# carpedkm/disentangled-subject-to-vid

Measured on AMD Instinct MI355X. Metric: denoise steps/sec (CogVideoX-5B, 49f 720x480; one step = CFG-pair transformer forward + CFG + scheduler step), higher is better.
Workload: dtype bf16

## Files before the change

disentangled-subject-to-vid_amd/csrc/api.hip:

```cpp
#define S2V_HOST
#include "common.h"
#include "kernels.h"
#include "../../include/s2v_hip.h"

#include <algorithm>
#include <cstdio>
#include <cstring>
#include <string>
#include <unordered_map>
#include <vector>

thread_local std::string g_s2v_err;
int s2v_fail(const char* file, int line, const char* msg, int code) {
    char buf[512];
    snprintf(buf, sizeof(buf), "%s:%d: %s", file, line, msg);
    g_s2v_err = buf;
    return code;
}

static inline int64_t rup(int64_t x, int64_t m) { return (x + m - 1) / m * m; }

struct Slot {
    char* dst = nullptr;
    int64_t rows = 0, cols = 0, ld = 0;
// ... 558 lines not shown
                for (int64_t j = 0; j < n; ++j, ++i) { omap[i] = (int)((so + j * Dp) / 16); omap[Mg + i] = (int)((so + n * Dp) / 4 + j * (Dp / 128)); }
            c->xcnt[1][0][g] = o_bytes(n); c->xcnt[1][1][g] = so; so += c->xcnt[1][0][g];
            c->xcnt[1][2][g] = o_bytes(c->M); c->xcnt[1][3][g] = g * o_bytes(c->M);
            c->xcnt[2][0][g] = (int64_t)B * c->Vmax * Cout4 * E; c->xcnt[2][1][g] = 0;
            c->xcnt[2][2][g] = c->xcnt[2][0][g]; c->xcnt[2][3][g] = g * c->xcnt[2][0][g];
        }
        if (omx) S2V_CHECK_HIP(hipMemcpy(c->omap, omap.data(), omap.size() * 4, hipMemcpyHostToDevice));
    }
    return 0;
}

extern "C" int s2v_fp8_qk_active(s2v_ctx* c, int32_t* active) {
    S2V_REQUIRE(c && active, "s2v_fp8_qk_active: null argument");
    *active = c->fp8_qk ? 1 : 0;
    return 0;
}

extern "C" int s2v_set_rope(s2v_ctx* c, const float* cos_dev, const float* sin_dev, s2v_stream stream) {
    S2V_REQUIRE(c && c->ws, "s2v_set_rope: call s2v_set_geometry first");
    auto drop_graph = [&]() { if (c->gexec) { hipGraphExecDestroy(c->gexec); c->gexec = nullptr; } };
    if (!cos_dev || !sin_dev) {
        if (c->have_rope) drop_graph();
        c->have_rope = false;
        return 0;
    }
    const bool had_rope = c->have_rope, was_paired = c->rope_paired;
    const size_t bytes = (size_t)(c->R + c->V) * 64 * 4;
    if (c->shard) {
        const size_t row = 64 * 4, rb = (size_t)c->R * row, vb = (size_t)c->V * row;
        const size_t ro = (size_t)c->r0 * row, vo = ((size_t)c->gR + c->v0) * row;
        S2V_CHECK_HIP(hipMemcpyAsync(c->rope_cos, (const char*)cos_dev + ro, rb, hipMemcpyDeviceToDevice, (hipStream_t)stream));
        S2V_CHECK_HIP(hipMemcpyAsync(c->rope_sin, (const char*)sin_dev + ro, rb, hipMemcpyDeviceToDevice, (hipStream_t)stream));
        S2V_CHECK_HIP(hipMemcpyAsync((char*)c->rope_cos + rb, (const char*)cos_dev + vo, vb, hipMemcpyDeviceToDevice, (hipStream_t)stream));
        S2V_CHECK_HIP(hipMemcpyAsync((char*)c->rope_sin + rb, (const char*)sin_dev + vo, vb, hipMemcpyDeviceToDevice, (hipStream_t)stream));
    } else {
        S2V_CHECK_HIP(hipMemcpyAsync(c->rope_cos, cos_dev, bytes, hipMemcpyDeviceToDevice, (hipStream_t)stream));
        S2V_CHECK_HIP(hipMemcpyAsync(c->rope_sin, sin_dev, bytes, hipMemcpyDeviceToDevice, (hipStream_t)stream));
    }
    c->have_rope = true;
    const size_t n = (size_t)(c->R + c->V) * 64;
    std::vector<float> hc(n), hs(n), pk(n);
    S2V_CHECK_HIP(hipStreamSynchronize((hipStream_t)stream));
    S2V_CHECK_HIP(hipMemcpy(hc.data(), c->rope_cos, bytes, hipMemcpyDeviceToHost));
    S2V_CHECK_HIP(hipMemcpy(hs.data(), c->rope_sin, bytes, hipMemcpyDeviceToHost));
    bool paired = true;
    for (size_t i = 0; i < n && paired; i += 2) paired = hc[i] == hc[i + 1] && hs[i] == hs[i + 1];
    c->rope_paired = paired;
    if (!had_rope || was_paired != paired) drop_graph();
    if (paired) {
        for (size_t p = 0; p < n / 64; ++p)
            for (int k = 0; k < 32; ++k) {
                pk[p * 64 + k] = hc[p * 64 + 2 * k];
                pk[p * 64 + 32 + k] = hs[p * 64 + 2 * k];
            }
        S2V_CHECK_HIP(hipMemcpy(c->rope_pk, pk.data(), bytes, hipMemcpyHostToDevice));
    }
    return 0;
}

extern "C" int s2v_set_pos_embed(s2v_ctx* c, const void* table_dev, s2v_stream stream) {
    S2V_REQUIRE(c && c->ws, "s2v_set_pos_embed: call s2v_set_geometry first");
    if (!table_dev) { c->have_pos = false; return 0; }
    S2V_CHECK_HIP(hipMemcpyAsync(c->pos_tab, (const char*)table_dev + (size_t)c->v0 * c->D * c->esz, (size_t)c->V * c->D * c->esz,
                                 hipMemcpyDeviceToDevice, (hipStream_t)stream));
    c->have_pos = true;
    return 0;
}

static int linear(s2v_ctx* c, const GemmArgs& g0, int epi, hipStream_t st) {
    GemmArgs g = g0;
    g.clk = c->clk_cur;
    g.a_rows_padded = (int)(rup(g.M, 256));
    g.w_rows_padded = (int)(rup(g.N, 256));
    if ((c->mfma || c->h16) && g.K % 64 == 0 && g.lda % 8 == 0 && g.ldw % 8 == 0) {
        g.f16 = c->h16 ? 1 : 0;
        const GemmPlan p = gemm_plan(g, epi, c->num_cus, c->sk_tiles);
        g.tile = p.tile;
        if (p.splitk > 1) { g.splitk = p.splitk; g.sk_ws = c->sk_ws; g.sk_cnt = c->sk_cnt; }
        if (p.tail != GEMM_NONE) {
            GemmArgs gm = g, gt = g;
            gt.clk = nullptr;
            gm.M = p.m_main;
            gt.m_begin = p.m_main;
            S2V_CHECK_HIP(hipEventRecord(c->ev_fork, st));
            S2V_CHECK_HIP(hipStreamWaitEvent(c->side, c->ev_fork, 0));
            S2V_TRY(launch_gemm_bf16(gt, epi, c->side));
            S2V_CHECK_HIP(hipEventRecord(c->ev_join, c->side));
            S2V_TRY(launch_gemm_bf16(gm, epi, st));
            S2V_CHECK_HIP(hipStreamWaitEvent(st, c->ev_join, 0));
            return 0;
        }
        return launch_gemm_bf16(g, epi, st);
    }
    g.valu_only = c->cfg.force_simple;
    return launch_gemm_simple(g, epi, c->dtype, st);
}

static int linear_fp8(s2v_ctx* c, const GemmArgs& g0, int epi, const char* wq, const float* wscale, hipStream_t st, bool prequant = false) {
    GemmArgs g = g0;
    g.clk = c->clk_cur;
    g.a_scale = nullptr;
    if (!g.mx_a_s) {
        if (!prequant) S2V_TRY(launch_quant_rows_fp8(g.A, g.lda, g.M, g.K, c->aq, c->aq_scale, st));
        g.A = c->aq; g.a_scale = c->aq_scale;
    }
    g.lda = g.K; g.W = wq; g.ldw = g.K; g.w_scale = wscale;
    g.a_rows_padded = (int)rup(g.M, 256);
    g.w_rows_padded = (int)rup(g.N, 256);
    return launch_gemm_fp8(g, epi, st);
}

extern "C" int s2v_set_conditioning(s2v_ctx* c, const void* text_dev, const void* ref_latent_dev, s2v_stream stream) {
    S2V_REQUIRE(c && c->ws && c->finalized, "s2v_set_conditioning: geometry and weights must be set first");
    S2V_REQUIRE(text_dev && ref_latent_dev, "s2v_set_conditioning: null input");
    hipStream_t st = (hipStream_t)stream;
    const int D = c->D;
    const int TX = c->cfg.text_embed_dim;
    if (c->T > 0) {
        if (c->shard) {
            for (int b = 0; b < c->B; ++b)
                S2V_TRY(launch_convert2d((const char*)text_dev + ((int64_t)b * c->gT + c->t0) * TX * c->esz, c->dtype, TX,
                                         c->Hb + (int64_t)b * c->T * TX * c->esz, c->dtype, TX, c->T, TX, st));
        } else {
            S2V_TRY(launch_convert2d(text_dev, c->dtype, TX, c->Hb, c->dtype, TX, (int64_t)c->B * c->T, TX, st));
        }
        GemmArgs g{};
        g.A = c->Hb; g.lda = TX; g.W = c->text_w; g.ldw = TX; g.bias = c->text_b;
        g.C = c->e0; g.ldc = D; g.M = c->B * c->T; g.N = D; g.K = TX;
        S2V_TRY(linear(c, g, EPI_BIAS, st));
    }
    const int K = c->cfg.in_channels * 4;
    S2V_TRY(launch_patchify(ref_latent_dev, 0, 1, 1, c->cfg.in_channels, c->H, c->W, c->patches, c->dtype, st));
    GemmArgs g{};
    g.A = c->patches + (int64_t)c->r0 * K * c->esz; g.lda = K; g.W = c->patch_w; g.ldw = K; g.bias = c->patch_b;
    g.C = c->e1; g.ldc = D; g.M = c->R; g.N = D; g.K = K;
    if (c->R > 0) S2V_TRY(linear(c, g, EPI_BIAS, st));
    c->have_cond = true;
    return 0;
}

#ifdef S2V_DIAG
static int g_fp8_mx = 1;
extern "C" __attribute__((visibility("default"))) int s2v_set_fp8_mx(int on) { g_fp8_mx = on; return 0; }
static int g_fused_q8 = 1;
extern "C" __attribute__((visibility("default"))) int s2v_set_fused_q8(int on) { g_fused_q8 = on; return 0; }
static int g_fused_qk = 1;
extern "C" __attribute__((visibility("default"))) int s2v_set_fused_qk(int on) { g_fused_qk = on; return 0; }
extern "C" __attribute__((visibility("default"))) int s2v_diag_qkv_qknorm(const void* A, const void* W, const void* bias, const void* nq_w, const void* nq_b,
                                                                           const void* nk_w, const void* nk_b, const float* cs, void* C, int32_t M, int32_t D,
                                                                           int32_t K, int32_t tok_per_batch, int32_t text_len, float eps, s2v_stream stream) {
    S2V_REQUIRE(A && W && bias && C && nq_w && nq_b && nk_w && nk_b, "s2v_diag_qkv_qknorm: null argument");
    GemmArgs g{};
    g.A = A; g.lda = K; g.W = W; g.ldw = K; g.bias = bias; g.C = C; g.ldc = 3 * D; g.M = M; g.N = 3 * D; g.K = K;
    g.a_rows_padded = (int)rup(M, 256); g.w_rows_padded = (int)rup(3 * D, 256);
    g.tok_per_batch = tok_per_batch; g.text_len = text_len;
    g.qk_w[0] = nq_w; g.qk_b[0] = nq_b; g.qk_w[1] = nk_w; g.qk_b[1] = nk_b; g.qk_cs = cs; g.qk_D = D; g.qk_eps = eps;
    return launch_gemm_bf16(g, EPI_BIAS_QKNORM, (hipStream_t)stream);
}
#endif
static bool attn_mx_out(const s2v_ctx* c) {
    bool mx = c->fp8 && c->mfma && c->D % 128 == 0;
#ifdef S2V_DIAG
    mx = mx && g_fp8_mx;
#endif
    return mx;
}
static int run_attention(s2v_ctx* c, int l, hipStream_t st, bool prequant = false) {
    const LayerW& w = c->layers[l];
    const int D = c->D;
    GemmArgs g{};
    g.A = c->Xn; g.lda = D; g.W = w.wqkv; g.ldw = D; g.bias = w.bqkv;
// ... 909 lines not shown
```

disentangled-subject-to-vid_amd/csrc/gemm.hip:

```cpp
#define S2V_HOST
#include "common.h"
#include "kernels.h"
#include <type_traits>
#include <algorithm>
#include <cstdlib>

#include "gemm_epi.h"
#include "epi_dispatch.h"

#define BM 128
#define BN 128
#define BK 64
#define TILE_BYTES (BM * BK * 2)

__device__ __forceinline__ int64_t a_row_base(const GemmArgs& a, int m) {
    if (!a.conv) return (int64_t)m * a.lda;
    m = min(m, a.M - 1);
    const int hw = a.oH * a.oW;
    const int f = m / hw, rem = m - f * hw;
    const int y = rem / a.oW, x = rem - y * a.oW;
    const int cs = a.cstride > 1 ? a.cstride : 1;
    return (((int64_t)f * a.Hp + y * cs) * a.Wp + x * cs) * a.cin;
}
__device__ __forceinline__ int64_t a_k_off(const GemmArgs& a, int k) {
// ... 49 lines not shown
template <int EPI, typename T16 = bf16_t>
__global__ __launch_bounds__(256, 2) void gemm_bf16_128(const GemmArgs a, int tiles_m, int tiles_n) {
    extern __shared__ __attribute__((aligned(16))) char smem[];
    const int tid = threadIdx.x, lane = tid & 63, wave = tid >> 6;
    const int wm = wave >> 1, wn = wave & 1;

    const int nwg = gridDim.x, bid = blockIdx.x;
    const int q = nwg >> 3, r = nwg & 7, xcd = bid & 7, idx = bid >> 3;
    const int wg = (xcd < r ? xcd * (q + 1) : r * (q + 1) + (xcd - r) * q) + idx;
    const int GM = 8;
    const int per_group = GM * tiles_n;
    const int group = wg / per_group;
    const int first_m = group * GM;
    const int gsz = min(tiles_m - first_m, GM);
    const int in_g = wg - group * per_group;
    const int tile_m = first_m + in_g % gsz;
    const int tile_n = in_g / gsz;
    const int m0 = a.m_begin + tile_m * BM, n0 = tile_n * BN;

    const bf16_t* A = (const bf16_t*)a.A;
    const bf16_t* W = (const bf16_t*)a.W;

    f32x16 acc[2][2];
#pragma unroll
    for (int i = 0; i < 2; ++i)
#pragma unroll
        for (int j = 0; j < 2; ++j)
#pragma unroll
            for (int e = 0; e < 16; ++e) acc[i][j][e] = 0.f;

    const int nt = a.K / BK;
    int64_t rb[4];
#pragma unroll
    for (int i = 0; i < 4; ++i) rb[i] = a_row_base(a, m0 + ((i * 256 + tid) >> 3));
    stage_tile_a(A, rb, a_k_off(a, 0), smem, tid);
    stage_tile(W, a.ldw, n0, 0, smem + TILE_BYTES, tid);
    __syncthreads();

    const int fr = lane & 31, hi = lane >> 5;
    for (int t = 0; t < nt; ++t) {
        const int cur = t & 1;
        if (t + 1 < nt) {
            stage_tile_a(A, rb, a_k_off(a, (t + 1) * BK), smem + (cur ^ 1) * 2 * TILE_BYTES, tid);
            stage_tile(W, a.ldw, n0, (t + 1) * BK, smem + (cur ^ 1) * 2 * TILE_BYTES + TILE_BYTES, tid);
        }
        const char* tA = smem + cur * 2 * TILE_BYTES;
        const char* tW = tA + TILE_BYTES;
#pragma unroll
        for (int kk = 0; kk < 4; ++kk) {
            bf16x8 wf[2], af[2];
#pragma unroll
            for (int i = 0; i < 2; ++i) wf[i] = lds_frag(tW, wn * 64 + i * 32 + fr, kk * 2 + hi);
#pragma unroll
            for (int j = 0; j < 2; ++j) af[j] = lds_frag(tA, wm * 64 + j * 32 + fr, kk * 2 + hi);
#pragma unroll
            for (int i = 0; i < 2; ++i)
#pragma unroll
                for (int j = 0; j < 2; ++j) {
                    if constexpr (std::is_same<T16, f16_t>::value)
                        acc[i][j] = __builtin_amdgcn_mfma_f32_32x32x16_f16(__builtin_bit_cast(f16x8, wf[i]), __builtin_bit_cast(f16x8, af[j]), acc[i][j], 0, 0, 0);
                    else
                        acc[i][j] = __builtin_amdgcn_mfma_f32_32x32x16_bf16(wf[i], af[j], acc[i][j], 0, 0, 0);
                }
        }
        __syncthreads();
    }

    if (epi_vec_ok(a, EPI)) {
        epilogue_wave<EPI, 2, false, T16>(a, acc, m0 + wm * 64, n0 + wn * 64, smem + wave * 8192, lane);
        return;
    }
#pragma unroll
    for (int i = 0; i < 2; ++i)
#pragma unroll
        for (int j = 0; j < 2; ++j) {
            const int m = m0 + wm * 64 + j * 32 + fr;
#pragma unroll
            for (int rq = 0; rq < 4; ++rq) {
                const int n = n0 + wn * 64 + i * 32 + 8 * rq + 4 * hi;
                float v[4] = {acc[i][j][rq * 4 + 0], acc[i][j][rq * 4 + 1], acc[i][j][rq * 4 + 2], acc[i][j][rq * 4 + 3]};
                if (n < a.N) epilogue4<T16, EPI>(a, m, n, v);
            }
        }
}

bool gemm_f16_ok(const GemmArgs& a, int epi) {
    if (epi == EPI_BIAS_QKNORM || a.splitk > 1 || a.m_begin != 0) return false;
    if (a.K % BK != 0 || a.ldw % 8 != 0 || (a.conv ? a.cin % 64 != 0 : a.lda % 8 != 0)) return false;
    const int64_t mp = (int64_t)((a.M + BM - 1) / BM) * BM, np = (int64_t)((a.N + BN - 1) / BN) * BN;
    return (a.conv || a.a_rows_padded >= mp) && (a.w_rows_padded >= np || a.N % BN == 0);
}
int launch_gemm_f16(const GemmArgs& a0, int epi, hipStream_t st) {
    S2V_REQUIRE(gemm_f16_ok(a0, epi), "gemm_f16: shape / padding not supported");
    GemmArgs a = a0;
    a.f16 = 1;
    return launch_gemm_bf16(a, epi, st);
}

#define RBM 256
#define RBN 128
#define RA_BYTES (RBM * BK * 2)
#define RW_BYTES (RBN * BK * 2)
#define RSTAGE (RA_BYTES + RW_BYTES)

template <int EPI, typename T16 = bf16_t>
__global__ __launch_bounds__(512, 2) void gemm_bf16_stag(const GemmArgs a, int tiles_m, int tiles_n) {
    extern __shared__ __attribute__((aligned(16))) char smem[];
    const int tid = threadIdx.x, lane = tid & 63;
    const int wave = __builtin_amdgcn_readfirstlane(tid >> 6);
    const int grp = wave >> 2;
    const int wm = wave & 3, wn = grp;

    const int nwg = gridDim.x, bid = blockIdx.x;
    const int q = nwg >> 3, r = nwg & 7, xcd = bid & 7, idx = bid >> 3;
    const int wg = (xcd < r ? xcd * (q + 1) : r * (q + 1) + (xcd - r) * q) + idx;
    const int GM = 4;
    const int per_group = GM * tiles_n;
    const int group = wg / per_group;
    const int first_m = group * GM;
    const int gsz = min(tiles_m - first_m, GM);
    const int in_g = wg - group * per_group;
    const int m0 = (first_m + in_g % gsz) * RBM, n0 = (in_g / gsz) * RBN;

    const int64_t rbase0 = a_row_base(a, m0);
    const char* Abase = (const char*)a.A + 2 * rbase0;
    const char* Wbase = (const char*)a.W + 2 * (int64_t)n0 * a.ldw;
    unsigned offA[4], offW[2];
#pragma unroll
    for (int i = 0; i < 4; ++i) {
        const int gi = i * 512 + tid, row = gi >> 3;
        offA[i] = (unsigned)(2 * (a_row_base(a, m0 + row) - rbase0 + ((gi & 7) ^ ((row >> 1) & 7)) * 8));
    }
#pragma unroll
    for (int i = 0; i < 2; ++i) {
        const int gi = i * 512 + tid, row = gi >> 3;
        offW[i] = (unsigned)(2 * ((int64_t)row * a.ldw + ((gi & 7) ^ ((row >> 1) & 7)) * 8));
    }
    auto stage = [&](int t, int s) {
        char* base = smem + s * RSTAGE;
        const char* ta = Abase + 2 * a_k_off(a, t * BK);
        const char* tw = Wbase + 2 * (int64_t)t * BK;
#pragma unroll
        for (int i = 0; i < 4; ++i) glds16_saddr(ta, offA[i], base + (i * 512 + wave * 64) * 16);
#pragma unroll
        for (int i = 0; i < 2; ++i) glds16_saddr(tw, offW[i], base + RA_BYTES + (i * 512 + wave * 64) * 16);
    };

    f32x16 acc[2][2];
#pragma unroll
    for (int i = 0; i < 2; ++i)
#pragma unroll
        for (int j = 0; j < 2; ++j)
#pragma unroll
            for (int e = 0; e < 16; ++e) acc[i][j][e] = 0.f;
    bf16x8 wf[4][2], af[4][2];
    const int fr = lane & 31, hi = lane >> 5;

    auto load_frags = [&](int t) {
        const char* tA = smem + (t % 3) * RSTAGE;
        const char* tW = tA + RA_BYTES;
#pragma unroll
        for (int kk = 0; kk < 4; ++kk) {
#pragma unroll
            for (int i = 0; i < 2; ++i) wf[kk][i] = lds_frag(tW, wn * 64 + i * 32 + fr, kk * 2 + hi);
#pragma unroll
            for (int j = 0; j < 2; ++j) af[kk][j] = lds_frag(tA, wm * 64 + j * 32 + fr, kk * 2 + hi);
// ... 738 lines not shown
        if (blockIdx.x == 100 && lane == 0)
            for (int e = 0; e < 8; ++e) g_pp_dbg[wave * 8 + e] = tacc[e];
        if (tid == 0 && blockIdx.x < 256) {
            long long* o = g_blk_times + (launch_no & 1) * 1024 + blockIdx.x * 4;
            o[0] = tr0;
            o[1] = tr0 + tacc[6];
            o[2] = tacc[5];
            o[3] = tacc[7];
            if (blockIdx.x == 0) g_launch_no = launch_no + 1;
        }
    }
#endif
}

template <int EPI>
static int launch_q4_t(const GemmArgs& a, hipStream_t st) {
    const int tiles_m = (a.M + WBM - 1) / WBM, tiles_n = (a.N + WBN - 1) / WBN;
    const void* fn = (const void*)gemm_q4<EPI, 0>;
    if (EPI == EPI_BIAS) switch (a.ablate) {
            case 5: fn = (const void*)gemm_q4<EPI_BIAS, 2>; break;
            case 6: fn = (const void*)gemm_q4<EPI_BIAS, 2 | 4>; break;
            default: break;
        }
    S2V_TRY(ensure_lds_attr(fn, 163840));
    const int grid = std::min((device_cus() / 8) * 8, ((tiles_m * tiles_n + 7) / 8) * 8);
    void* args[] = {(void*)&a, (void*)&tiles_m, (void*)&tiles_n};
    S2V_CHECK_HIP(hipLaunchKernel(fn, dim3(grid), dim3(256), args, 163840, st));
    return 0;
}
#endif

int device_cus() {
    static int cus[64] = {0};
    int d = 0;
    if (hipGetDevice(&d) != hipSuccess || d < 0 || d >= 64) d = 0;
    if (!cus[d]) {
        int n = 0;
        if (hipDeviceGetAttribute(&n, hipDeviceAttributeMultiprocessorCount, d) != hipSuccess || n <= 0) n = 256;
        cus[d] = n;
    }
    return cus[d];
}

template <int EPI, typename T16 = bf16_t>
static int launch_pp64_t(const GemmArgs& a_in, hipStream_t st) {
    GemmArgs a = a_in;
    const int tiles_m = (a.M + WBM - 1) / WBM, tiles_n = (a.N + WBN - 1) / WBN;
    if (a.gm <= 0) a.gm = (!a.conv && tiles_n <= 16 && tiles_m >= 32) ? (a.K >= 8192 ? 1 : 3) : 4;
    S2V_TRY(ensure_lds_attr((const void*)gemm_bf16_pp64<EPI, 0, false, T16>, 131072));
#ifdef S2V_DIAG
    if (EPI == EPI_BIAS && a.ablate) {
        const void* fn = a.ablate == 1 ? (const void*)gemm_bf16_pp64<EPI_BIAS, 1> : a.ablate == 4 ? (const void*)gemm_bf16_pp64<EPI_BIAS, 4> : a.ablate == 5 ? (const void*)gemm_bf16_pp64<EPI_BIAS, 5> : a.ablate == 6 ? (const void*)gemm_bf16_pp64<EPI_BIAS, 6> : a.ablate == 7 ? (const void*)gemm_bf16_pp64<EPI_BIAS, 7> : (const void*)gemm_bf16_pp64<EPI_BIAS, 3>;
        S2V_CHECK_HIP(hipFuncSetAttribute(fn, hipFuncAttributeMaxDynamicSharedMemorySize, 131072));
        void* args[] = {(void*)&a, (void*)&tiles_m, (void*)&tiles_n};
        S2V_CHECK_HIP(hipLaunchKernel(fn, dim3(tiles_m * tiles_n), dim3(512), args, 131072, st));
        return 0;
    }
#endif
    hipLaunchKernelGGL((gemm_bf16_pp64<EPI, 0, false, T16>), dim3(tiles_m * tiles_n), dim3(512), 131072, st, a, tiles_m, tiles_n);
    S2V_CHECK_HIP(hipGetLastError());
    return 0;
}

#ifdef S2V_DIAG
template <int EPI>
static int launch_w8_t(const GemmArgs& a, hipStream_t st) {
    const int tiles_m = (a.M + WBM - 1) / WBM, tiles_n = (a.N + WBN - 1) / WBN;
    S2V_TRY(ensure_lds_attr((const void*)gemm_bf16_w8<EPI>, WH_NST * WH_STAGE));
    hipLaunchKernelGGL(gemm_bf16_w8<EPI>, dim3(tiles_m * tiles_n), dim3(512), WH_NST * WH_STAGE, st, a, tiles_m, tiles_n);
    S2V_CHECK_HIP(hipGetLastError());
    return 0;
}
#endif

template <int EPI, typename T16 = bf16_t>
static int launch_stag_t(const GemmArgs& a, hipStream_t st) {
    const int tiles_m = (a.M + RBM - 1) / RBM, tiles_n = (a.N + RBN - 1) / RBN;
    S2V_TRY(ensure_lds_attr((const void*)gemm_bf16_stag<EPI, T16>, 3 * RSTAGE));
    hipLaunchKernelGGL((gemm_bf16_stag<EPI, T16>), dim3(tiles_m * tiles_n), dim3(512), 3 * RSTAGE, st, a, tiles_m, tiles_n);
    S2V_CHECK_HIP(hipGetLastError());
    return 0;
}

template <int EPI, typename T16 = bf16_t>
static int launch_128_t(const GemmArgs& a, hipStream_t st) {
    const int tiles_m = (a.M - a.m_begin + BM - 1) / BM, tiles_n = (a.N + BN - 1) / BN;
    hipLaunchKernelGGL((gemm_bf16_128<EPI, T16>), dim3(tiles_m * tiles_n), dim3(256), 4 * TILE_BYTES, st, a, tiles_m, tiles_n);
    S2V_CHECK_HIP(hipGetLastError());
    return 0;
}

#ifdef S2V_DIAG
int g_gemm_ablate = 0;
int g_gemm_impl = 9;
int g_gemm_g4t = 1;
extern "C" __attribute__((visibility("default"))) int s2v_set_gemm_g4t(int on) { g_gemm_g4t = on; return 0; }
extern "C" __attribute__((visibility("default"))) int s2v_set_gemm_impl(int impl) { g_gemm_impl = impl & 0xff; g_gemm_ablate = impl >> 8; return 0; }
extern "C" __attribute__((visibility("default"))) int s2v_diag_gemm_plan(int32_t M, int32_t N, int32_t K, int32_t epi, int32_t flags, int32_t ncu,
                                                                          int64_t sk_tiles, int32_t* out) {
    S2V_REQUIRE(out && M > 0 && N > 0 && K > 0 && ncu > 0, "s2v_diag_gemm_plan: bad argument");
    static char p[16];
    GemmArgs g{};
    g.A = p; g.lda = K; g.W = p; g.ldw = K; g.bias = p; g.C = p; g.ldc = N; g.M = M; g.N = N; g.K = K;
    g.a_rows_padded = (M + 255) / 256 * 256; g.w_rows_padded = (N + 255) / 256 * 256;
    g.X = p; g.ldx = N; g.gate_vid = p; g.gate_txt = p; g.gate_stride = N; g.R = p; g.ldr = N;
    g.tok_per_batch = M; g.qk_w[0] = g.qk_w[1] = g.qk_b[0] = g.qk_b[1] = p; g.qk_D = N / 3; g.qk_cs = (flags & 2) ? (const float*)p : nullptr;
    g.f16 = flags & 1;
    if (flags & 4) {
        g.w_scale = (const float*)p;
        if (flags & 8) { g.mx_a_s = (const unsigned char*)p; g.mx_rows = g.a_rows_padded; }
        else g.a_scale = (const float*)p;
    }
    if (flags & 16) { g.conv = 1; g.kt = 3; g.cin = K / 27; g.lda = 0; g.a_rows_padded = 0; }
    const GemmPlan pl = gemm_plan(g, epi, ncu, sk_tiles);
    out[0] = pl.splitk; out[1] = pl.tile; out[2] = pl.m_main; out[3] = pl.main; out[4] = pl.tail;
    return 0;
}
#else
static constexpr int g_gemm_ablate = 0;
static constexpr int g_gemm_impl = 9;
static constexpr int g_gemm_g4t = 1;
#endif

template <int EPI>
static int launch_fp8_t(const GemmArgs& a, hipStream_t st) {
    const int tiles_m = (a.M + WBM - 1) / WBM, tiles_n = (a.N + WBN - 1) / WBN;
    S2V_TRY(ensure_lds_attr((const void*)gemm_bf16_pp64<EPI, 0, true>, 131072 + 2048));
    hipLaunchKernelGGL((gemm_bf16_pp64<EPI, 0, true>), dim3(tiles_m * tiles_n), dim3(512), 131072 + 2048, st, a, tiles_m, tiles_n);
    S2V_CHECK_HIP(hipGetLastError());
    return 0;
}

static bool w_tile_ok(const GemmArgs& a) {
    if (a.N % WBN == 0) return true;
    return a.N > WBN && a.w_rows_padded >= ((a.N + WBN - 1) / WBN) * WBN && (a.N % WBN) >= WBN / 2;
}
static bool fits_256(const GemmArgs& a) { return w_tile_ok(a) && (a.conv || a.a_rows_padded >= ((a.M + WBM - 1) / WBM) * WBM); }

static int gemm_kernel(const GemmArgs& a, int epi, int ncu) {
    if (a.w_scale) return g_gemm_impl == 9 && gemm_g4f_ok(a, epi) ? GEMM_G4F : GEMM_PP64_FP8;
    if (a.m_begin > 0 || (epi == EPI_BIAS_QKNORM && !fits_256(a))) return GEMM_128;
#ifdef S2V_DIAG
    if (g_gemm_impl == 8 && !a.conv && (epi == EPI_BIAS || epi == EPI_BIAS_GELU) && w_tile_ok(a) && a.N % 64 == 0 && a.K >= 36 * 64 &&
        epi_vec_ok(a, epi) && a.a_rows_padded >= ((a.M + WBM - 1) / WBM) * WBM && a.lda % 8 == 0 && a.ldw % 8 == 0)
        return GEMM_Q4;
#endif
    bool g4_epi = true, g4t_epi = true;
#ifdef S2V_DIAG
    if (const char* e = getenv("S2V_G4_EPI_MASK")) g4_epi = (atoi(e) >> epi) & 1;
    if (const char* e = getenv("S2V_G4T_EPI_MASK")) g4t_epi = (atoi(e) >> epi) & 1;
#endif
    const int64_t out_tiles = (int64_t)((a.M + 255) / 256) * ((a.N + 255) / 256);
    if (epi == EPI_BIAS_QKNORM && out_tiles <= ncu) g4_epi = false;
    if (epi == EPI_BIAS_GELU && a.splitk <= 1 && a.K <= 2048 && out_tiles <= 2 * ncu) g4_epi = false;
    const bool conv_few = a.conv && out_tiles * 2 <= ncu && epi != EPI_BIAS_QKNORM;
    const bool big_tiles = (a.tile == 0 && !conv_few) || (a.conv && !conv_few) || epi == EPI_BIAS_QKNORM;
    const bool g4 = g_gemm_impl == 9 && big_tiles && w_tile_ok(a) && gemm_g4_ok(a, epi);
    if (g4 && g_gemm_g4t && g4t_epi && !a.f16 && gemm_g4t_ok(a, epi, ncu)) return GEMM_G4T;
    if (g4 && g4_epi) return GEMM_G4;
    if ((g_gemm_impl == 7 || g_gemm_impl == 8 || g_gemm_impl == 9) && big_tiles && fits_256(a)) return GEMM_PP64;
#ifdef S2V_DIAG
    if (g_gemm_impl == 5 && fits_256(a)) return GEMM_W8;
#endif
    if ((g_gemm_impl == 2 || g_gemm_impl >= 4) && (a.tile != 2 || a.conv) && epi != EPI_BIAS_QKNORM && (a.conv || a.a_rows_padded >= ((a.M + RBM - 1) / RBM) * RBM))
        return GEMM_STAG;
    return GEMM_128;
}

GemmPlan gemm_plan(const GemmArgs& g0, int epi, int ncu, int64_t sk_tiles) {
    GemmArgs g = g0;
    int m_main = g.M;
    if (!g.conv && !g.w_scale) {
        const int64_t tn = (g.N + 255) / 256, tm = (g.M + 255) / 256;
        if (sk_tiles > 0 && g.splitk == 0) {
            const int S = gemm_choose_splitk(tm * tn, g.K, ncu);
            if (S > 1 && (int64_t)S * tm * tn <= sk_tiles) g.splitk = S;
        }
        if (g.splitk == 0 && epi != EPI_BIAS_QKNORM && g.tile == 0 && tm * tn * 2 <= ncu) g.tile = 1;
        if (g.M % 256 != 0 && tm > 1 && g.N >= 256) {
            GemmArgs gw = g;
            gw.M = (int)((tm - 1) * 256);
            if ((tm * tn + ncu - 1) / ncu > ((tm - 1) * tn + ncu - 1) / ncu || gemm_kernel(gw, epi, ncu) == GEMM_G4T) m_main = gw.M;
        }
    }
    GemmArgs gm = g, gt = g;
    gm.M = m_main;
    gt.m_begin = m_main;
    return GemmPlan{g.splitk, g.tile, m_main, gemm_kernel(gm, epi, ncu), m_main < g.M ? gemm_kernel(gt, epi, ncu) : (int)GEMM_NONE};
}

int launch_gemm_fp8(const GemmArgs& a, int epi, hipStream_t st) {
    S2V_REQUIRE(!a.conv && (a.a_scale || a.mx_a_s) && a.w_scale, "gemm_fp8: plain mode with the weight scales and row or block scales of A only");
    S2V_REQUIRE(!a.mx_out_q || (epi == EPI_BIAS_GELU && a.mx_out_s && a.N % 64 == 0), "gemm_fp8: MX output is the GELU epilogue's, N a multiple of 64");
    S2V_REQUIRE(!(a.mx_out_q || a.mx_a_s) || a.mx_rows >= ((a.M + WBM - 1) / WBM) * WBM, "gemm_fp8: MX block scales are K-tile major, mx_rows must cover the padded M");
    S2V_REQUIRE(a.K % 128 == 0 && a.lda % 16 == 0 && a.ldw % 16 == 0, "gemm_fp8: K must be a multiple of 128, rows 16-byte aligned");
    S2V_REQUIRE(a.a_rows_padded >= ((a.M + WBM - 1) / WBM) * WBM && a.w_rows_padded >= ((a.N + WBN - 1) / WBN) * WBN,
                "gemm_fp8: operands must be padded to whole 256-row tiles");
    S2V_REQUIRE(epi_vec_ok(a, epi), "gemm_fp8: output rows must be 16-byte aligned and N a multiple of 8");
    if (gemm_kernel(a, epi, 0) == GEMM_G4F) return launch_gemm_g4f(a, epi, st);
    return epi_dispatch<EPI_BIAS, EPI_BIAS_GELU, EPI_BIAS_GATE_RES, EPI_BIAS_QKNORM>(epi, "gemm_fp8: bad epilogue",
                                                                                   [&](auto e) { return launch_fp8_t<decltype(e)::value>(a, st); });
}

int launch_gemm_bf16(const GemmArgs& a0, int epi, hipStream_t st) {
    GemmArgs a = a0;
    a.ablate = g_gemm_ablate;
    S2V_REQUIRE(epi != EPI_BIAS_QKNORM || (!a.conv && epi_vec_ok(a, epi) && a.qk_D > 0 && a.qk_D % 64 == 0 && a.N == 3 * a.qk_D && a.tok_per_batch > 0 &&
                                           a.qk_w[0] && a.qk_w[1] && a.qk_b[0] && a.qk_b[1]),
                "gemm_bf16: fused qk-norm needs the vector epilogue, N = 3 * qk_D and the LayerNorm parameters");
    const int k = gemm_kernel(a, epi, device_cus());
    if (a.m_begin > 0) {
        S2V_REQUIRE(!a.conv && a.K % BK == 0 && a.lda % 8 == 0 && a.ldw % 8 == 0, "gemm_bf16: bad tail launch");
    } else if (epi != EPI_BIAS_QKNORM || fits_256(a)) {
        S2V_REQUIRE(a.K % BK == 0, "gemm_bf16: K must be a multiple of 64");
        S2V_REQUIRE(!a.f16 || (a.splitk <= 1 && a.mx_out_q == nullptr), "gemm (fp16): no split K or MX output");
        if (k == GEMM_PP64 || k == GEMM_W8 || k == GEMM_STAG || k == GEMM_128)
            S2V_REQUIRE((a.conv ? a.cin % 64 == 0 : a.lda % 8 == 0) && a.ldw % 8 == 0, "gemm_bf16: bad leading dims");
    }
    switch (k) {
#ifdef S2V_DIAG
        case GEMM_Q4: return epi_dispatch<EPI_BIAS, EPI_BIAS_GELU>(epi, "gemm_bf16: bad epilogue", [&](auto e) { return launch_q4_t<decltype(e)::value>(a, st); });
        case GEMM_W8:
            return epi_dispatch<EPI_BIAS, EPI_BIAS_GELU, EPI_BIAS_GATE_RES, EPI_BIAS_ADD>(epi, "gemm_bf16: bad epilogue",
                                                                                          [&](auto e) { return launch_w8_t<decltype(e)::value>(a, st); });
#endif
        case GEMM_G4T: return launch_gemm_g4t(a, epi, st);
        case GEMM_G4: return launch_gemm_g4(a, epi, st);
        case GEMM_PP64:
            return epi_dispatch16<EPI_BIAS, EPI_BIAS_GELU, EPI_BIAS_GATE_RES, EPI_BIAS_ADD, EPI_BIAS_QKNORM>(
                epi, a.f16, "gemm_bf16: bad epilogue", [&](auto e, auto t) { return launch_pp64_t<decltype(e)::value, decltype(t)>(a, st); });
        case GEMM_STAG:
            return epi_dispatch16<EPI_BIAS, EPI_BIAS_GELU, EPI_BIAS_GATE_RES, EPI_BIAS_ADD>(
                epi, a.f16, "gemm_bf16: bad epilogue", [&](auto e, auto t) { return launch_stag_t<decltype(e)::value, decltype(t)>(a, st); });
        default:
            return epi_dispatch16<EPI_BIAS, EPI_BIAS_GELU, EPI_BIAS_GATE_RES, EPI_BIAS_ADD, EPI_BIAS_QKNORM>(
                epi, a.f16, "gemm_bf16: bad epilogue", [&](auto e, auto t) { return launch_128_t<decltype(e)::value, decltype(t)>(a, st); });
    }
}

template <typename T, int EPI>
__global__ __launch_bounds__(256) void gemm_simple_k(const GemmArgs a) {
    __shared__ float sA[16][64 + 4];
    __shared__ float sW[16][64 + 4];
    const int tid = threadIdx.x;
    const int m0 = blockIdx.y * 64, n0 = blockIdx.x * 64;
    const int tm = (tid >> 4) * 4, tn = (tid & 15) * 4;
    const T* A = (const T*)a.A;
    const T* W = (const T*)a.W;
    float acc[4][4] = {};
    for (int k0 = 0; k0 < a.K; k0 += 16) {
#pragma unroll
        for (int i = 0; i < 4; ++i) {
            const int e = i * 256 + tid;
            const int row = e >> 4, k = e & 15;
            float va = 0.f, vw = 0.f;
            if (k0 + k < a.K) {
                if (m0 + row < a.M) va = ET<T>::ld(A + a_row_base(a, m0 + row) + a_k_off(a, k0 + k));
                if (n0 + row < a.N) vw = ET<T>::ld(W + (size_t)(n0 + row) * a.ldw + k0 + k);
            }
            sA[k][row] = va;
            sW[k][row] = vw;
        }
        __syncthreads();
#pragma unroll
        for (int k = 0; k < 16; ++k) {
            float av[4], wv[4];
#pragma unroll
            for (int i = 0; i < 4; ++i) av[i] = sA[k][tm + i];
#pragma unroll
            for (int j = 0; j < 4; ++j) wv[j] = sW[k][tn + j];
#pragma unroll
            for (int i = 0; i < 4; ++i)
#pragma unroll
                for (int j = 0; j < 4; ++j) acc[i][j] = fmaf(av[i], wv[j], acc[i][j]);
        }
        __syncthreads();
    }
#pragma unroll
    for (int i = 0; i < 4; ++i) {
        if (n0 + tn < a.N) epilogue4<T, EPI>(a, m0 + tm + i, n0 + tn, acc[i]);
    }
}

template <typename T>
static int launch_simple_t(const GemmArgs& a, int epi, hipStream_t st) {
    dim3 grid((a.N + 63) / 64, (a.M + 63) / 64);
    return epi_dispatch<EPI_BIAS, EPI_BIAS_GELU, EPI_BIAS_GATE_RES, EPI_BIAS_ADD>(epi, "gemm_simple: bad epilogue", [&](auto e) {
        hipLaunchKernelGGL((gemm_simple_k<T, decltype(e)::value>), grid, dim3(256), 0, st, a);
        S2V_CHECK_HIP(hipGetLastError());
        return 0;
    });
}

int launch_gemm_simple(const GemmArgs& a, int epi, int dtype, hipStream_t st) {
    if (dtype == S2V_F32 && gemm_f32m_ok(a)) return launch_gemm_f32m(a, epi, st);
    S2V_REQUIRE((a.M + 63) / 64 <= 65535, "gemm_simple: M too large for the generic kernel");
    S2V_DT_DISPATCH(dtype, return launch_simple_t<T>(a, epi, st))
    return 0;
}

__global__ void gemm_strided_f32_k(const float* A, int64_t sam, int64_t sak, const float* B, int64_t sbn, int64_t sbk,
                                   float* C, int64_t ldc, int M, int N, int K, float alpha) {
    const int n = blockIdx.x * blockDim.x + threadIdx.x;
    const int m = blockIdx.y;
    if (n >= N || m >= M) return;
    float acc = 0.f;
    for (int k = 0; k < K; ++k) acc = fmaf(A[m * sam + k * sak], B[n * sbn + k * sbk], acc);
    C[m * ldc + n] += alpha * acc;
}
int launch_gemm_strided_f32(const float* A, int64_t sam, int64_t sak, const float* B, int64_t sbn, int64_t sbk,
                            float* C, int64_t ldc, int M, int N, int K, float alpha, hipStream_t st) {
    dim3 grid((N + 255) / 256, M);
    hipLaunchKernelGGL(gemm_strided_f32_k, grid, dim3(256), 0, st, A, sam, sak, B, sbn, sbk, C, ldc, M, N, K, alpha);
    S2V_CHECK_HIP(hipGetLastError());
    return 0;
}
```

disentangled-subject-to-vid_amd/csrc/kernels.h:

```cpp
#pragma once
#include <hip/hip_runtime.h>
#include <stdint.h>

enum { S2V_F32 = 0, S2V_BF16 = 1, S2V_F16 = 2 };
#define S2V_DT_DISPATCH(dtype, ...)                                        \
    switch (dtype) {                                                       \
        case S2V_BF16: { using T = bf16_t; __VA_ARGS__; } break;           \
        case S2V_F16: { using T = f16_t; __VA_ARGS__; } break;             \
        default: { using T = float; __VA_ARGS__; } break;                  \
    }
enum { EPI_BIAS = 0, EPI_BIAS_GELU = 1, EPI_BIAS_GATE_RES = 2 };

struct GemmArgs {
    const void* A; int lda;
    const void* W; int ldw;
    const void* bias;
    void* C; int ldc;
    int M, N, K;
    void* X; int ldx;
    const void* gate_vid; const void* gate_txt; int gate_stride;
    int tok_per_batch; int text_len;
    const void* gate_ref; int ref_len;
    const void* R; int ldr;
    int conv, cin, Hp, Wp, oH, oW, kt;
    int cstride;
    int gm;
    int tile;
    int ablate;
    long long* clk;
    int f16;
    int valu_only;
    int a_rows_padded;
    int m_begin;
    int w_rows_padded;
    const float* a_scale;
    const float* w_scale;
    const void* qk_w[2]; const void* qk_b[2];
    const float* qk_cs;
    int qk_D; float qk_eps;
    int splitk; float* sk_ws; unsigned* sk_cnt;
    unsigned char* mx_out_q; unsigned char* mx_out_s;
    const unsigned char* mx_a_s;
    int mx_rows;
};
int launch_gemm_fp8(const GemmArgs& a, int epi, hipStream_t st);
int launch_quant_rows_fp8(const void* src, int64_t ld, int64_t M, int K, void* dst, float* scale, hipStream_t st);
enum { EPI_BIAS_ADD = 3 };
enum { EPI_BIAS_QKNORM = 4 };

__host__ __device__ __forceinline__ int64_t mx_perm_row(int64_t m) { return (m & ~(int64_t)127) | ((m & 31) << 2) | ((m >> 5) & 3); }
int launch_gemm_bf16(const GemmArgs& a, int epi, hipStream_t st);
int launch_gemm_simple(const GemmArgs& a, int epi, int dtype, hipStream_t st);
bool gemm_f16_ok(const GemmArgs& a, int epi);
int launch_gemm_f16(const GemmArgs& a, int epi, hipStream_t st);
bool gemm_f32m_ok(const GemmArgs& a);
int launch_gemm_f32m(const GemmArgs& a, int epi, hipStream_t st);
bool gemm_g4_ok(const GemmArgs& a, int epi);
int launch_gemm_g4(const GemmArgs& a, int epi, hipStream_t st);
bool gemm_g4f_ok(const GemmArgs& a, int epi);
int launch_gemm_g4f(const GemmArgs& a, int epi, hipStream_t st);
bool gemm_g4t_ok(const GemmArgs& a, int epi, int ncu);
int launch_gemm_g4t(const GemmArgs& a, int epi, hipStream_t st);
int gemm_choose_splitk(int64_t tiles, int K, int64_t ncu);
int device_cus();
enum GemmKernel { GEMM_NONE = 0, GEMM_128, GEMM_STAG, GEMM_PP64, GEMM_G4, GEMM_G4T, GEMM_W8, GEMM_Q4, GEMM_G4F, GEMM_PP64_FP8 };
struct GemmPlan {
    int splitk;
    int tile;
    int m_main;
    int main;
    int tail;
};
GemmPlan gemm_plan(const GemmArgs& g, int epi, int ncu, int64_t sk_tiles);
int launch_gemm_strided_f32(const float* A, int64_t sam, int64_t sak, const float* B, int64_t sbn, int64_t sbk,
                            float* C, int64_t ldc, int M, int N, int K, float alpha, hipStream_t st);

struct AttnArgs {
    const void* qkv; int ld_qkv;
    const void* vt;
    int ntok_pad;
    void* out; int ld_out;
    int B, H, Ntok;
    float scale;
    int* queue; int num_cus;
    unsigned char* mx_q; unsigned char* mx_s; int mx_rows;
    const unsigned char* q8; const unsigned short* q8s; const unsigned char* k8; const unsigned* k8s;
    int p16;
    unsigned long long* stats;
    long long* clk;
    int order;
    int stagger;
    int valu_only;
};
#ifndef ATTN_PP_MAX_TOKENS
#define ATTN_PP_MAX_TOKENS 4608
#endif
static inline bool attn_runs_q4(int Ntok, bool mx_out) { return mx_out || Ntok > ATTN_PP_MAX_TOKENS; }
int launch_qk_quant_mx(const void* qkv, int ld_qkv, int B, int H, int Ntok, int ntok_pad, float q_prescale, unsigned char* q8, unsigned short* q8s,
                       unsigned char* k8, unsigned* k8s, hipStream_t st);
struct QkNormRopeArgs;
int launch_qk_norm_quant_mx(const QkNormRopeArgs& a, float q_prescale, unsigned char* q8, unsigned short* q8s, unsigned char* k8, unsigned* k8s, hipStream_t st);
int launch_attn_q4f(const AttnArgs& a, bool persistent, hipStream_t st);
int launch_attn_q4h(const AttnArgs& a, bool persistent, hipStream_t st);
int launch_attn_bf16(const AttnArgs& a, hipStream_t st);
int launch_attn_simple(const AttnArgs& a, int dtype, hipStream_t st);
int launch_attn_f32m(const AttnArgs& a, int dtype, hipStream_t st);
int launch_attn_f16(const AttnArgs& a, hipStream_t st);
int launch_attn_q4hh(const AttnArgs& a, bool persistent, hipStream_t st);
int launch_attn_q4(const AttnArgs& a, bool persistent, hipStream_t st);
int launch_attn_q8(const AttnArgs& a, bool persistent, hipStream_t st);

struct LnModArgs {
    const void* x; int ldx; void* y; int ldy;
    const void* w; const void* b; float eps;
    const void* shift_vid; const void* scale_vid; const void* shift_txt; const void* scale_txt; int mod_stride;
    int B, Ntok, text_len, D;
    const void* shift_ref; const void* scale_ref; int ref_len;
    void* q8; float* q8_scale;
};
int launch_ln_modulate(const LnModArgs& a, int dtype, hipStream_t st);

struct QkNormRopeArgs {
    void* qkv; int ld_qkv; int B, H, Ntok, text_len;
    const void* nq_w; const void* nq_b; const void* nk_w; const void* nk_b; float eps;
    const float* cos; const float* sin;
    void* vt; int ntok_pad;
    int vt_f16;
};
int launch_qk_norm_rope(const QkNormRopeArgs& a, int dtype, hipStream_t st);
int launch_v_transpose(const void* qkv, int ld_qkv, int B, int H, int Ntok, void* vt, int ntok_pad, hipStream_t st, bool to_f16 = false);

int launch_time_embed(const float* t_dev, int B, int D, const void* w1, const void* b1, const void* w2, const void* b2,
                      int temb_dim, void* tmp , void* emb_out , int dtype, hipStream_t st);
int launch_mod_gemv(const void* emb, int B, int temb_dim, const void* W, const void* bias, int64_t rows_total,
                    void* out , int dtype, hipStream_t st, bool rowwise = false);

int launch_patchify(const void* lat, int64_t lat_bstride, int Bn, int F, int C, int H, int W, void* out, int dtype,
                    hipStream_t st);
int launch_unpatchify(const void* y, int ldy, int64_t y_bstride, void* out, int B, int F, int C, int H, int W, int dtype,
                      hipStream_t st);
struct ShardCopyArgs {
    const char* src; char* dst;
    int rows, width16;
    int64_t src_ld, dst_ld;
    const int* src_map; const int* dst_map;
    int nseg, nseg_inner;
    int64_t src_seg_outer, src_seg_inner, dst_seg_outer, dst_seg_inner;
};
int launch_shard_copy(const ShardCopyArgs& a, hipStream_t st);
struct ShardScaleArgs {
    const unsigned* src; unsigned* dst;
    int rows, nkt, nseg;
    const int* src_map; const int* dst_map;
    int64_t src_row, src_kt, src_seg, dst_row, dst_kt, dst_seg;
    int src_perm, dst_perm;
};
// ... 34 lines not shown
```

Before: 1.618.

## Add narrow-N tail GEMM kernel and choose tail placement by main kernel

Adds a 128x64-tile GEMM kernel with a four-stage pipeline, used for the leftover M rows of a split GEMM. It launches twice as many tiles along N, so the small tail fills more CUs. The tail's placement now depends on the main kernel. Tails run serially after the main GEMM unless the main kernel is G4T, which keeps the side-stream fork. This drops the event and fork overhead, and the risk of slowing the main kernel through contention, but gives up overlap for non-G4T main kernels.

```diff
diff --git a/disentangled-subject-to-vid_amd/csrc/api.hip b/disentangled-subject-to-vid_amd/csrc/api.hip
--- a/disentangled-subject-to-vid_amd/csrc/api.hip
+++ b/disentangled-subject-to-vid_amd/csrc/api.hip
@@ -664,11 +664,17 @@
             gt.clk = nullptr;
             gm.M = p.m_main;
             gt.m_begin = p.m_main;
+            const int place = gemm_tail_place(p);
+            if (place == TAIL_AFTER) {
+                S2V_TRY(launch_gemm_bf16(gm, epi, st));
+                return launch_gemm_bf16(gt, epi, st);
+            }
             S2V_CHECK_HIP(hipEventRecord(c->ev_fork, st));
             S2V_CHECK_HIP(hipStreamWaitEvent(c->side, c->ev_fork, 0));
+            if (place == TAIL_FORK_MAIN_FIRST) S2V_TRY(launch_gemm_bf16(gm, epi, st));
             S2V_TRY(launch_gemm_bf16(gt, epi, c->side));
             S2V_CHECK_HIP(hipEventRecord(c->ev_join, c->side));
-            S2V_TRY(launch_gemm_bf16(gm, epi, st));
+            if (place != TAIL_FORK_MAIN_FIRST) S2V_TRY(launch_gemm_bf16(gm, epi, st));
             S2V_CHECK_HIP(hipStreamWaitEvent(st, c->ev_join, 0));
             return 0;
         }
diff --git a/disentangled-subject-to-vid_amd/csrc/gemm.hip b/disentangled-subject-to-vid_amd/csrc/gemm.hip
--- a/disentangled-subject-to-vid_amd/csrc/gemm.hip
+++ b/disentangled-subject-to-vid_amd/csrc/gemm.hip
@@ -155,6 +155,89 @@
                 if (n < a.N) epilogue4<T16, EPI>(a, m, n, v);
             }
         }
+}
+
+#define TBN 64
+#define TNS 4
+#define TA_BYTES (BM * BK * 2)
+#define TW_BYTES (TBN * BK * 2)
+#define TSTAGE (TA_BYTES + TW_BYTES)
+template <int EPI, typename T16 = bf16_t>
+__global__ __launch_bounds__(256, 1) void gemm_bf16_tail(const GemmArgs a, int tiles_n) {
+    extern __shared__ __attribute__((aligned(16))) char smem[];
+    const int tid = threadIdx.x, lane = tid & 63;
+    const int wave = __builtin_amdgcn_readfirstlane(tid >> 6);
+    const int tile_m = blockIdx.x / tiles_n, tile_n = blockIdx.x - tile_m * tiles_n;
+    const int m0 = a.m_begin + tile_m * BM, n0 = tile_n * TBN;
+
+    const char* Abase = (const char*)a.A + 2 * (int64_t)m0 * a.lda;
+    const char* Wbase = (const char*)a.W + 2 * (int64_t)n0 * a.ldw;
+    unsigned offA[4], offW[2];
+#pragma unroll
+    for (int i = 0; i < 4; ++i) {
+        const int gi = i * 256 + tid, row = gi >> 3;
+        offA[i] = (unsigned)(2 * ((int64_t)row * a.lda + ((gi & 7) ^ ((row >> 1) & 7)) * 8));
+    }
+#pragma unroll
+    for (int i = 0; i < 2; ++i) {
+        const int gi = i * 256 + tid, row = gi >> 3;
+        offW[i] = (unsigned)(2 * ((int64_t)row * a.ldw + ((gi & 7) ^ ((row >> 1) & 7)) * 8));
+    }
+    const unsigned lds0 = lds_base_u32(smem);
+    auto stage = [&](int t) {
+        const unsigned base = lds0 + (t % TNS) * TSTAGE;
+        const char* ta = Abase + 2 * (int64_t)t * BK;
+        const char* tw = Wbase + 2 * (int64_t)t * BK;
+#pragma unroll
+        for (int i = 0; i < 4; ++i) glds16_saddr_m0(ta, offA[i], base + (i * 256 + wave * 64) * 16);
+#pragma unroll
+        for (int i = 0; i < 2; ++i) glds16_saddr_m0(tw, offW[i], base + TA_BYTES + (i * 256 + wave * 64) * 16);
+    };
+
+    f32x16 acc[2][1];
+#pragma unroll
+    for (int i = 0; i < 2; ++i)
+#pragma unroll
+        for (int e = 0; e < 16; ++e) acc[i][0][e] = 0.f;
+
+    const int nt = a.K / BK;
+    for (int t = 0; t < TNS - 1 && t < nt; ++t) stage(t);
+    const int fr = lane & 31, hi = lane >> 5;
+    for (int t = 0; t < nt; ++t) {
+        static_assert(TNS == 4, "the counted waits below are written for four stages");
+        const int younger = min(nt - 1 - t, TNS - 2);
+        if (younger >= 2) asm volatile("s_waitcnt vmcnt(12) lgkmcnt(0)\n\ts_barrier" ::: "memory");
+        else if (younger == 1) asm volatile("s_waitcnt vmcnt(6) lgkmcnt(0)\n\ts_barrier" ::: "memory");
+        else asm volatile("s_waitcnt vmcnt(0) lgkmcnt(0)\n\ts_barrier" ::: "memory");
+        if (t + TNS - 1 < nt) stage(t + TNS - 1);
+        const char* tA = smem + (t % TNS) * TSTAGE;
+        const char* tW = tA + TA_BYTES;
+#pragma unroll
+        for (int kk = 0; kk < 4; ++kk) {
+            bf16x8 wf[2];
+#pragma unroll
+            for (int i = 0; i < 2; ++i) wf[i] = lds_frag(tW, i * 32 + fr, kk * 2 + hi);
+            const bf16x8 af = lds_frag(tA, wave * 32 + fr, kk * 2 + hi);
+#pragma unroll
+            for (int i = 0; i < 2; ++i) acc[i][0] = mfma16<T16>(wf[i], af, acc[i][0]);
+        }
+    }
+    asm volatile("s_waitcnt lgkmcnt(0)\n\ts_barrier" ::: "memory");
+
+    if (epi_vec_ok(a, EPI)) {
+        epilogue_wave<EPI, 1, false, T16>(a, acc, m0 + wave * 32, n0, smem + wave * 4096, lane);
+        return;
+    }
+#pragma unroll
+    for (int i = 0; i < 2; ++i) {
+        const int m = m0 + wave * 32 + fr;
+#pragma unroll
+        for (int rq = 0; rq < 4; ++rq) {
+            const int n = n0 + i * 32 + 8 * rq + 4 * hi;
+            float v[4] = {acc[i][0][rq * 4 + 0], acc[i][0][rq * 4 + 1], acc[i][0][rq * 4 + 2], acc[i][0][rq * 4 + 3]};
+            if (n < a.N) epilogue4<T16, EPI>(a, m, n, v);
+        }
+    }
 }
 
 bool gemm_f16_ok(const GemmArgs& a, int epi) {
@@ -1059,9 +1142,38 @@
     return 0;
 }
 
+#ifdef S2V_DIAG
+int g_gemm_tail_narrow = -1;
+int g_gemm_tail_place = -1;
+extern "C" __attribute__((visibility("default"))) int s2v_set_gemm_tail(int narrow, int place) { g_gemm_tail_narrow = narrow; g_gemm_tail_place = place; return 0; }
+static int diag_knob(int v, const char* env, int dflt) {
+    if (v >= 0) return v;
+    const char* e = getenv(env);
+    return e ? atoi(e) : dflt;
+}
+#endif
+
+static bool tail_narrow_ok(const GemmArgs& a, int epi) {
+#ifdef S2V_DIAG
+    if (!diag_knob(g_gemm_tail_narrow, "S2V_GEMM_TAIL_NARROW", 1)) return false;
+#endif
+    if (a.m_begin <= 0 || a.conv || a.mx_out_q || !(epi == EPI_BIAS || epi == EPI_BIAS_GELU || epi == EPI_BIAS_GATE_RES)) return false;
+    const int64_t mp = a.m_begin + (int64_t)((a.M - a.m_begin + BM - 1) / BM) * BM, np = (int64_t)((a.N + TBN - 1) / TBN) * TBN;
+    return a.K % BK == 0 && a.lda % 8 == 0 && a.ldw % 8 == 0 && a.a_rows_padded >= mp && (a.N % TBN == 0 || a.w_rows_padded >= np);
+}
+
 template <int EPI, typename T16 = bf16_t>
 static int launch_128_t(const GemmArgs& a, hipStream_t st) {
     const int tiles_m = (a.M - a.m_begin + BM - 1) / BM, tiles_n = (a.N + BN - 1) / BN;
+    if constexpr (EPI == EPI_BIAS || EPI == EPI_BIAS_GELU || EPI == EPI_BIAS_GATE_RES) {
+        if (tail_narrow_ok(a, EPI)) {
+            const int tn = (a.N + TBN - 1) / TBN;
+            S2V_TRY(ensure_lds_attr((const void*)gemm_bf16_tail<EPI, T16>, TNS * TSTAGE));
+            hipLaunchKernelGGL((gemm_bf16_tail<EPI, T16>), dim3(tiles_m * tn), dim3(256), TNS * TSTAGE, st, a, tn);
+            S2V_CHECK_HIP(hipGetLastError());
+            return 0;
+        }
+    }
     hipLaunchKernelGGL((gemm_bf16_128<EPI, T16>), dim3(tiles_m * tiles_n), dim3(256), 4 * TILE_BYTES, st, a, tiles_m, tiles_n);
     S2V_CHECK_HIP(hipGetLastError());
     return 0;
@@ -1166,6 +1278,14 @@
     return GemmPlan{g.splitk, g.tile, m_main, gemm_kernel(gm, epi, ncu), m_main < g.M ? gemm_kernel(gt, epi, ncu) : (int)GEMM_NONE};
 }
 
+int gemm_tail_place(const GemmPlan& p) {
+#ifdef S2V_DIAG
+    const int v = diag_knob(g_gemm_tail_place, "S2V_GEMM_TAIL_PLACE", -1);
+    if (v >= 0) return v;
+#endif
+    return p.main == GEMM_G4T ? TAIL_FORK : TAIL_AFTER;
+}
+
 int launch_gemm_fp8(const GemmArgs& a, int epi, hipStream_t st) {
     S2V_REQUIRE(!a.conv && (a.a_scale || a.mx_a_s) && a.w_scale, "gemm_fp8: plain mode with the weight scales and row or block scales of A only");
     S2V_REQUIRE(!a.mx_out_q || (epi == EPI_BIAS_GELU && a.mx_out_s && a.N % 64 == 0), "gemm_fp8: MX output is the GELU epilogue's, N a multiple of 64");
@@ -1215,6 +1335,26 @@
     }
 }
 
+#ifdef S2V_DIAG
+extern "C" __attribute__((visibility("default"))) int s2v_diag_linear_rows(const void* A, const void* W, const void* bias, void* C, void* X,
+                                                                            const void* gate, int32_t M, int32_t N, int32_t K, int32_t epi,
+                                                                            int32_t m_begin, int32_t rows_padded, int32_t narrow, void* stream) {
+    S2V_REQUIRE(A && W && bias && M > 0 && N % 256 == 0 && K % 64 == 0 && m_begin >= 0 && m_begin < M && rows_padded >= (M + 255) / 256 * 256,
+                "s2v_diag_linear_rows: bad argument");
+    S2V_REQUIRE(epi == EPI_BIAS_GATE_RES ? (X && gate) : (C && (epi == EPI_BIAS || epi == EPI_BIAS_GELU)), "s2v_diag_linear_rows: bad epilogue");
+    GemmArgs g{};
+    g.A = A; g.lda = K; g.W = W; g.ldw = K; g.bias = bias; g.C = C; g.ldc = N; g.M = M; g.N = N; g.K = K;
+    g.a_rows_padded = rows_padded; g.w_rows_padded = N;
+    g.X = X; g.ldx = N; g.gate_vid = gate; g.gate_txt = gate; g.gate_stride = N; g.tok_per_batch = M;
+    g.m_begin = m_begin;
+    const int keep = g_gemm_tail_narrow;
+    g_gemm_tail_narrow = narrow ? 1 : 0;
+    const int rc = launch_gemm_bf16(g, epi, (hipStream_t)stream);
+    g_gemm_tail_narrow = keep;
+    return rc;
+}
+#endif
+
 template <typename T, int EPI>
 __global__ __launch_bounds__(256) void gemm_simple_k(const GemmArgs a) {
     __shared__ float sA[16][64 + 4];
diff --git a/disentangled-subject-to-vid_amd/csrc/kernels.h b/disentangled-subject-to-vid_amd/csrc/kernels.h
--- a/disentangled-subject-to-vid_amd/csrc/kernels.h
+++ b/disentangled-subject-to-vid_amd/csrc/kernels.h
@@ -72,6 +72,8 @@
     int tail;
 };
 GemmPlan gemm_plan(const GemmArgs& g, int epi, int ncu, int64_t sk_tiles);
+enum GemmTailPlace { TAIL_FORK = 0, TAIL_AFTER = 1, TAIL_FORK_MAIN_FIRST = 2 };
+int gemm_tail_place(const GemmPlan& p);
 int launch_gemm_strided_f32(const float* A, int64_t sam, int64_t sak, const float* B, int64_t sbn, int64_t sbk,
                             float* C, int64_t ldc, int M, int N, int K, float alpha, hipStream_t st);
 
```

Result: no change. 1.628 (median of 6 runs) (+0.7%).
